# KhaoulaAguech/pl-fem-vectoriel

Hardware: AMD Instinct MI355X
Metric: eigenmodes/sec (assembly+solve), 7-core P2 mesh, 10 modes; |Δn_eff| vs ref (higher is better)
Workload: dtype f64

## Files before the change

pl_fem_vectoriel_amd/csrc/api_device.hip:

```cpp
#include <algorithm>
#include <atomic>
#include <memory>
#include <cmath>
#include <cstdio>
#include <cstdlib>
#include <cstring>
#include <chrono>
#include <mutex>
#include <numeric>
#include <thread>
#include <vector>

#include "device.h"
#include "host_eig.h"
#include "p2_element.h"

using plfem::Symbolic;

namespace {
template <class T>
T& process_wide() {
  static T* t = new T();
  return *t;
}
// ... 523 lines not shown
  if (!c) return PLFEM_EINVAL;
  if (!c->assembled) { c->err = "plfem_factor before plfem_assemble_hfield"; return PLFEM_ESTATE; }
  HIP_TRY(c, hipSetDevice(c->device));
  TRY(wait_for_upload(c));
  HIP_TRY(c, phase_begin(c, plfem::PH_FACTOR));
  HIP_TRY(c, hipMemsetAsync(c->d_fvec, 0, sizeof(double) * 2 * c->fnodes_total * plfem::BLOCK_P, c->stream));
  plfem::launch_factor(c, sigma);
  if (c->test_post_factor) c->test_post_factor(c);
  HIP_TRY(c, phase_end(c, plfem::PH_FACTOR));
  TRY(check_launch(c, "factor"));
  c->sigma = sigma;
  c->factored = true;
  return PLFEM_OK;
} catch (...) { return host_failure(c); }

extern "C" int plfem_solve(plfem_ctx* c, const double* rhs_dev, double* x_dev, int32_t refine_steps) try {
  if (!c || !rhs_dev || !x_dev || refine_steps < 0) return PLFEM_EINVAL;
  if (!c->factored) { c->err = "plfem_solve before plfem_factor"; return PLFEM_ESTATE; }
  HIP_TRY(c, hipSetDevice(c->device));
  plfem::solve_refined(c, 1, rhs_dev, x_dev, c->n2, false, refine_steps, c->d_t1, c->d_t2, c->d_t2);
  return check_launch(c, "solve");
} catch (...) { return host_failure(c); }

namespace {
struct ThickRestart {
  plfem_ctx* c;
  int P, k, ld;
  double tol;
  double* hH;
  std::vector<double> T, Tm, theta, Svec;
  std::vector<int> order;
  int nconv = 0, restarts = 0;
  double max_rel_res = 0.0;

  ThickRestart(plfem_ctx* c_, int P_, int k_, int m, double tol_)
      : c(c_), P(P_), k(k_), ld(m + P_), tol(tol_), hH(c_->h_pinned + plfem::PIN_PROJ), T((size_t)ld * ld, 0.0) {}

  void fill_tm(int mm) {
    Tm.assign((size_t)mm * mm, 0.0);
    for (int j = 0; j < mm; ++j)
      for (int i = 0; i <= j; ++i) {
        const double v = T[(size_t)j * ld + i];
        Tm[(size_t)j * mm + i] = v;
        Tm[(size_t)i * mm + j] = v;
      }
  }
  template <class Last>
  void count_converged(int mm, Last last) {
    order.resize(mm);
    std::iota(order.begin(), order.end(), 0);
    std::sort(order.begin(), order.end(), [&](int a, int b) { return std::fabs(theta[a]) > std::fabs(theta[b]); });
    nconv = 0;
    max_rel_res = 0.0;
    for (int q = 0; q < std::min(k, mm); ++q) {
      const int id = order[q];
      double res;
      if (P == 1) {
        res = std::fabs(T[(size_t)(mm - 1) * ld + mm] * last(id, 0));
      } else {
        double r2 = 0.0;
        for (int a = 0; a < P; ++a) {
          double v = 0.0;
          for (int b = a; b < P; ++b) v += T[(size_t)(mm - P + b) * ld + (mm + a)] * last(id, b);
          r2 += v * v;
        }
        res = std::sqrt(r2);
// ... 29 lines not shown
    std::swap(c->d_BV, c->d_BV2);
    std::fill(T.begin(), T.end(), 0.0);
    for (int q = 0; q < pk; ++q) T[(size_t)q * ld + q] = theta[order[q]];
    HIP_TRY(c, hipMemsetAsync(c->d_Hcols, 0, sizeof(double) * ld * ld, st));
    ++restarts;
    return PLFEM_OK;
  }

  int finish(int mm, double sigma, double* evals_host, double* evecs_dev, double* stats_host, int nop, int nblock) {
    hipStream_t st = c->stream;
    std::vector<int> want(order.begin(), order.begin() + k);
    std::vector<double> lam(mm);
    for (int i = 0; i < mm; ++i) lam[i] = sigma + 1.0 / theta[i];
    std::sort(want.begin(), want.end(), [&](int a, int b) { return lam[a] < lam[b]; });
    bool purify = nconv >= k;
    for (int a = 0; a < P; ++a) purify = purify && T[(size_t)(mm - P + a) * ld + (mm + a)] > 0.0;
    const int rows = purify ? mm + P : mm;
    for (int q = 0; q < k; ++q) {
      const int id = want[q];
      evals_host[q] = lam[id];
      double* s = hH + (size_t)q * rows;
      std::memcpy(s, &Svec[(size_t)id * mm], sizeof(double) * mm);
      for (int a = 0; a < rows - mm; ++a) {
        double v = 0.0;
        for (int b = a; b < P; ++b) v += T[(size_t)(mm - P + b) * ld + (mm + a)] * Svec[(size_t)id * mm + (mm - P + b)];
        s[mm + a] = v / theta[id];
      }
    }
    HIP_TRY(c, hipMemcpyAsync(c->d_S, hH, sizeof(double) * rows * k, hipMemcpyHostToDevice, st));
    if (!evecs_dev) evecs_dev = c->d_V2;
    c->modes_dev = evecs_dev;
    c->modes_k = k;
    plfem::launch_rotate(c, c->d_V, rows, c->d_S, rows, k, evecs_dev);
    HIP_TRY(c, phase_end(c, plfem::PH_LANCZOS));
    TRY(check_launch(c, "ritz rotation"));
    if (!c->defer_sync) HIP_TRY(c, hipStreamSynchronize(st));
    if (stats_host) {
      const double s[5] = {(double)nconv, (double)nop, (double)restarts, max_rel_res, (double)nblock};
      std::copy(s, s + 5, stats_host);
    }
    if (nconv < k) { c->err = "Lanczos: no convergence within maxiter restarts"; return PLFEM_ENOCONV; }
    return PLFEM_OK;
  }
};
}

static int lanczos_block(plfem_ctx* c, int k, int ncv, double tol, int maxiter, double sigma, double* evals_host,
                         double* evecs_dev, double* stats_host) {
  constexpr int P = plfem::BLOCK_P;
  const int64_t n = c->n2;
  hipStream_t st = c->stream;
  HIP_TRY(c, phase_begin(c, plfem::PH_LANCZOS));
  int m = ((ncv + P - 1) / P) * P;
  if (m > c->max_ncv) m = (c->max_ncv / P) * P;
  ThickRestart R(c, P, k, m, tol);
  const int ld = R.ld;
  int nop = 0, nblock = 0;
  {
    plfem::launch_start_field(c, P, c->d_V2);
    plfem::launch_spmv(c, 1, P, c->d_V2, c->d_bw, n);
    plfem::launch_solve(c, P, c->d_bw, c->d_w, n);
    nop += P; ++nblock;
    plfem::launch_spmv(c, 1, P, c->d_w, c->d_bw, n);
    plfem::launch_panel_dot(c, P, c->d_w, P, c->d_bw, n, c->d_G, P);
    plfem::launch_chol_block(c, c->d_G, P, c->d_hblk, P, c->d_Rinv);
    plfem::launch_block_scale(c, c->d_w, c->d_bw, n, c->d_Rinv, c->d_V, c->d_BV, n, nullptr, 0, nullptr, nullptr, c->d_fvec);
// ... 59 lines not shown
      R.ritz(mm_);
      return;
    }
    R.fill_tm(mm_);
    plfem::sym_band_eigenvalues(mm_, P, R.Tm.data(), mm_, R.theta);
    std::vector<int> ids(mm_);
    std::iota(ids.begin(), ids.end(), 0);
    std::sort(ids.begin(), ids.end(), [&](int a, int b) { return std::fabs(R.theta[a]) > std::fabs(R.theta[b]); });
    ids.resize(std::min(k, mm_));
    R.Svec.resize((size_t)mm_ * mm_);
    plfem::sym_band_eigenvectors(mm_, P, R.Tm.data(), mm_, R.theta, ids, R.Svec.data(), mm_);
    R.count_from_svec(mm_);
  };
  double res_prev = 0.0, res_last = 0.0;
  while (true) {
    int pend_c0 = -1, pend_slot = 0, slot = 0;
    bool converged = false, inflight = false, force_launch = false, have_full = false;
    mm = c0;
    while (true) {
      const bool predicted = !force_launch && pend_c0 >= 0 && res_prev > 0.0 && res_last > 0.0 &&
                             res_last * (res_last / res_prev) <= tol;
      force_launch = false;
      int new_c0 = -1, new_slot = 0;
      if (c0 + P <= m && !predicted) {
        TRY(launch_step(c0, slot));
        nop += P; ++nblock;
        new_c0 = c0; new_slot = slot;
        c0 += P; slot ^= 1;
      }
      if (pend_c0 >= 0) {
        TRY(absorb_step(pend_c0, pend_slot));
        mm = pend_c0 + P;
        if (mm >= k + P && (new_c0 >= 0 || predicted)) {
          if (predicted) { full_check(mm, false); have_full = true; } else { quick_check(mm); have_full = false; }
          res_prev = res_last;
          res_last = R.max_rel_res;
          if (getenv("PLFEM_LANCZOS_TRACE"))
            fprintf(stderr, "[lanczos] cols %d nconv %d max_rel_res %.3e%s\n", mm, R.nconv, R.max_rel_res, predicted ? " (held)" : "");
          if (R.nconv >= k) { converged = true; inflight = new_c0 >= 0; break; }
        }
        if (predicted) {
          pend_c0 = -1;
          force_launch = true;
          if (c0 + P <= m) continue;
          break;
        }
      }
      pend_c0 = new_c0; pend_slot = new_slot;
      if (pend_c0 < 0) break;
    }
    if (converged) {
      if (!have_full) full_check(mm, false);
      if (R.nconv < k) {
        converged = false;
        if (inflight) { TRY(absorb_step(c0 - P, slot ^ 1)); }
        res_prev = res_last = 0.0;
        if (c0 + P <= m) continue;
        mm = c0;
        full_check(mm, true);
      }
    } else {
      mm = c0;
      full_check(mm, true);
    }
    res_prev = res_last = 0.0;
    if (R.nconv >= k || R.restarts >= maxiter) break;
    int pk = 0;
    TRY(R.restart(mm, pk));
    c0 = pk;
    cycle_start = pk;
    il_ready = -1;
// ... 74 lines not shown
  if (!c || !evals_host || !evecs_dev) return PLFEM_EINVAL;
  return lanczos_run(c, k, ncv, tol, maxiter, sigma, evals_host, evecs_dev, stats_host);
} catch (...) { return host_failure(c); }

extern "C" int plfem_postprocess(plfem_ctx* c, int32_t k, double* evecs_dev, const double* cores_host, int32_t ncore,
                                 double* out_host, double* frac_core_host, double* modes_int_dev) try {
  if (!c || !evecs_dev || !out_host || k < 1 || k > c->max_ncv) return PLFEM_EINVAL;
  if (!c->assembled) { c->err = "plfem_postprocess before plfem_assemble_hfield"; return PLFEM_ESTATE; }
  HIP_TRY(c, hipSetDevice(c->device));
  TRY(upload_cores(c, cores_host, ncore));
  HIP_TRY(c, phase_begin(c, plfem::PH_POST));
  plfem::launch_post(c, k, evecs_dev, ncore, out_host, frac_core_host, modes_int_dev);
  HIP_TRY(c, phase_end(c, plfem::PH_POST));
  TRY(check_launch(c, "postprocess"));
  HIP_TRY(c, hipStreamSynchronize(c->stream));
  return PLFEM_OK;
} catch (...) { return host_failure(c); }

extern "C" int plfem_solve_modes(plfem_ctx* c, const double* cores_host, int32_t ncore, double eps_core, double eps_clad,
                                 double k0, double alpha_p, double sigma, int32_t k, int32_t ncv, double tol,
                                 int32_t maxiter, double residual_tol, double tol_refined, double* evals_host,
                                 double* post_host, double* frac_core_host, double* resid_host, double* modes_int_host,
                                 double* stats_host) try {
  if (!c || !evals_host || !post_host || !resid_host) return PLFEM_EINVAL;
  if (k < 1 || k > c->max_ncv) { c->err = "plfem_solve_modes: need 1 <= k <= max_ncv"; return PLFEM_EINVAL; }
  const double th0 = now_ms();
  HIP_TRY(c, hipSetDevice(c->device));
  if (!c->copy_stream) HIP_TRY(c, copy_stream_acquire(c->device, &c->copy_stream));
  if (!c->ev_copy) HIP_TRY(c, ctx_event_acquire(c->device, EV_NO_TIMING, &c->ev_copy));
  struct Defer {
    plfem_ctx* c;
    int saved_refine;
    bool copy_pending = false;
    hipEvent_t tr_ev[3] = {nullptr, nullptr, nullptr};
    ~Defer() {
      if (copy_pending) (void)hipStreamSynchronize(c->copy_stream);
      for (hipEvent_t e : tr_ev) if (e) (void)hipEventDestroy(e);
      c->defer_sync = false;
      c->refine_steps = saved_refine;
    }
  } defer{c, c->refine_steps};
  c->defer_sync = true;
  static const bool call_trace = getenv("PLFEM_CALL_TRACE") != nullptr;
  auto& tr_ev = defer.tr_ev;
  double th_asm = 0, th_fac = 0, th_lan = 0, th_enq = 0, th_sync = 0;
  if (call_trace) {
    for (auto& e : tr_ev) (void)hipEventCreate(&e);
    (void)hipEventRecord(tr_ev[0], c->stream);
  }
  if (c->dpn == 2) TRY(plfem_assemble_hfield(c, cores_host, ncore, eps_core, eps_clad, k0, alpha_p));
  else TRY(plfem_assemble_scalar(c, cores_host, ncore, eps_core, eps_clad, k0));
  th_asm = now_ms();
  TRY(plfem_factor(c, sigma));
  th_fac = now_ms();
  double st[8] = {0, 0, 0, 0, 0, 0, 0, 0};
  double first_res = 0.0, res = 0.0;
  int perturbed = 0, refined = 0;
  double n_opinv = 0, n_block = 0, restarts = 0;
  auto put_stats = [&](int lo, int hi) {
    if (!stats_host) return;
    double v[PLFEM_SOLVE_STATS] = {st[0], n_opinv, restarts, st[3], n_block, first_res, res, (double)refined, (double)perturbed};
    if (hi > PLFEM_SOLVE_T_ASSEMBLE_US) {
      for (int ph = 0; ph < plfem::PH_COUNT; ++ph) v[PLFEM_SOLVE_T_ASSEMBLE_US + ph] = phase_us(c, (plfem::Phase)ph);
      v[PLFEM_SOLVE_T_CALL_US] = (now_ms() - th0) * 1e3;
    }
    for (int q = lo; q < hi; ++q) stats_host[q] = v[q];
  };
  for (int pass = 0; pass < 2; ++pass) {
    c->refine_steps = pass == 0 ? defer.saved_refine : std::max(1, defer.saved_refine + 1);
    const double tol_p = pass == 0 ? tol : std::min(tol, tol_refined);
    const int rc = lanczos_run(c, k, ncv, tol_p, maxiter, sigma, evals_host, nullptr, st);
    n_opinv += st[1]; n_block += st[4]; restarts += st[2];
    if (rc != PLFEM_OK) {
      (void)hipStreamSynchronize(c->stream);
      put_stats(0, PLFEM_SOLVE_RESIDUAL_FIRST);
      return rc;
    }
    th_lan = now_ms();
    double* modes = c->modes_dev;
    double* modes_int = c->d_BV2 != modes ? c->d_BV2 : c->d_BV;
    HIP_TRY(c, phase_begin(c, plfem::PH_POST));
    hipError_t copy_err = hipSuccess;
    const size_t row_bytes = sizeof(double) * (size_t)c->dpn * c->nsolve;
    const std::function<void(int, int)> send_group = [&](int g0, int kg) {
      if (copy_err != hipSuccess) return;
      defer.copy_pending = true;
      copy_err = hipEventRecord(c->ev_copy, c->stream);
      if (copy_err == hipSuccess) copy_err = hipStreamWaitEvent(c->copy_stream, c->ev_copy, 0);
      if (copy_err == hipSuccess)
        copy_err = hipMemcpyAsync(reinterpret_cast<char*>(modes_int_host) + g0 * row_bytes, reinterpret_cast<char*>(modes_int) + g0 * row_bytes,
                                  kg * row_bytes, hipMemcpyDeviceToHost, c->copy_stream);
    };
    plfem::post_enqueue(c, k, modes, ncore, modes_int_host ? modes_int : nullptr, modes_int_host ? &send_group : nullptr);
    HIP_TRY(c, phase_end(c, plfem::PH_POST));
    HIP_TRY(c, copy_err);
    HIP_TRY(c, phase_begin(c, plfem::PH_RESIDUAL));
    plfem::resid_enqueue(c, k, evals_host, modes);
    HIP_TRY(c, phase_end(c, plfem::PH_RESIDUAL));
    TRY(check_launch(c, "post-processing + residual check"));
    if (call_trace) {
      (void)hipEventRecord(tr_ev[1], c->stream);
      (void)hipEventRecord(tr_ev[2], c->copy_stream);
    }
    th_enq = now_ms();
    HIP_TRY(c, hipStreamSynchronize(c->stream));
    th_sync = now_ms();
    plfem::post_finish(c, k, post_host, frac_core_host);
    plfem::resid_finish(c, k, resid_host);
    perturbed = reinterpret_cast<const int32_t*>(c->h_pinned + plfem::PIN_COUNTERS)[0];
    res = 0.0;
    for (int i = 0; i < k; ++i) res = (resid_host[i] > res || !(resid_host[i] == resid_host[i])) ? resid_host[i] : res;
    if (pass == 0) first_res = res;
    if (res <= residual_tol && perturbed == 0) break;
    if (modes_int_host) HIP_TRY(c, hipStreamSynchronize(c->copy_stream));
    defer.copy_pending = false;
    if (pass == 1) {
      if (res <= residual_tol) break;
      char msg[512];
      std::snprintf(msg, sizeof(msg), "eigen-residual %.2e after the refined re-run (first pass %.2e, bound %.0e); %s", res, first_res,
                    residual_tol, perturbed > 0 ? "vanishing pivots were perturbed: the shift-invert factorisation is inaccurate on this mesh"
                                                : "no pivot was perturbed: the eigenpairs did not converge tightly enough");
      c->err = msg;
      put_stats(PLFEM_SOLVE_RESIDUAL_FIRST, PLFEM_SOLVE_T_ASSEMBLE_US);
      return PLFEM_ERESIDUAL;
    }
    refined = 1;
  }
  if (modes_int_host) HIP_TRY(c, hipStreamSynchronize(c->copy_stream));
  defer.copy_pending = false;
  if (call_trace) {
    const double th_end = now_ms();
    float backlog = 0, total = 0, copy_tail = 0;
    (void)hipEventElapsedTime(&backlog, tr_ev[0], c->ev[plfem::PH_ASSEMBLE][0]);
    (void)hipEventElapsedTime(&total, tr_ev[0], tr_ev[1]);
    (void)hipEventElapsedTime(&copy_tail, tr_ev[1], tr_ev[2]);
    fprintf(stderr, "[call] host: assemble enqueued +%.3f, factor +%.3f, lanczos returned +%.3f, post + check enqueued +%.3f, stream done +%.3f, "
                    "copy done +%.3f ms | device: entry -> assembly %.3f (backlog of plfem_create + launch), entry -> end of check %.3f, "
                    "check -> copy end %.3f ms\n",
            th_asm - th0, th_fac - th0, th_lan - th0, th_enq - th0, th_sync - th0, th_end - th0, backlog, total, copy_tail);
  }
  put_stats(0, PLFEM_SOLVE_STATS);
  return PLFEM_OK;
} catch (...) { return host_failure(c); }

extern "C" int plfem_modes_dev(plfem_ctx* c, const double** evecs_dev, int32_t* k) try {
  if (!c || !evecs_dev) return PLFEM_EINVAL;
  if (!c->modes_dev) { c->err = "plfem_modes_dev: no eigen-solve has run on this context"; return PLFEM_ESTATE; }
  *evecs_dev = c->modes_dev;
  if (k) *k = c->modes_k;
  return PLFEM_OK;
} catch (...) { return host_failure(c); }

extern "C" int plfem_timings(plfem_ctx* c, double* out_host) try {
  if (!c || !out_host) return PLFEM_EINVAL;
  HIP_TRY(c, hipStreamSynchronize(c->stream));
  int32_t cnt[4] = {0, 0, 0, 0};
  HIP_TRY(c, hipMemcpy(cnt, c->d_counters, sizeof(cnt), hipMemcpyDeviceToHost));
  for (int ph = plfem::PH_ASSEMBLE; ph <= plfem::PH_UPLOAD; ++ph) out_host[ph] = phase_us(c, (plfem::Phase)ph);
  out_host[5] = cnt[0];
  out_host[6] = phase_us(c, plfem::PH_RESIDUAL);
  out_host[7] = 0.0;
  return PLFEM_OK;
} catch (...) { return host_failure(c); }

extern "C" int plfem_profile_begin(plfem_ctx* c, int32_t max_ranges) try {
  if (!c || max_ranges < 1) return PLFEM_EINVAL;
  HIP_TRY(c, hipSetDevice(c->device));
  c->prof_max = max_ranges;
  if (c->prof_ev.empty()) process_wide<EventPool>().take_all(c->device, EV_PROFILE, c->prof_ev);
  c->prof_n = 0;
  c->prof_toggle = 0;
  c->prof_slot.clear();
// ... 48 lines not shown
```

pl_fem_vectoriel_amd/csrc/host_eig.cpp:

```cpp
#include "host_eig.h"

#include <cmath>
#include <algorithm>
#include <cstddef>
#include <cstdint>
#include <numeric>
#include <utility>

namespace plfem {

namespace {

bool ql_implicit(int n, double* w, double* e, double* Z, int np) {
  auto zrow = [&](int i) -> double* { return Z + (size_t)i * np; };
  for (int i = 1; i < n; ++i) e[i - 1] = e[i];
  e[n - 1] = 0.0;
  bool ok = true;
  for (int l = 0; l < n; ++l) {
    int iter = 0, m;
    do {
      for (m = l; m < n - 1; ++m) {
        double dd = std::fabs(w[m]) + std::fabs(w[m + 1]);
        if (std::fabs(e[m]) <= 2.3e-16 * dd) break;
      }
// ... 2 lines not shown
        double gq = (w[l + 1] - w[l]) / (2.0 * e[l]);
        double r = std::hypot(gq, 1.0);
        gq = w[m] - w[l] + e[l] / (gq + (gq >= 0.0 ? std::fabs(r) : -std::fabs(r)));
        double s = 1.0, c = 1.0, pp = 0.0;
        int i;
        for (i = m - 1; i >= l; --i) {
          double f = s * e[i], b = c * e[i];
          e[i + 1] = (r = std::sqrt(f * f + gq * gq));
          if (r == 0.0) {
            w[i + 1] -= pp;
            e[m] = 0.0;
            break;
          }
          s = f / r;
          c = gq / r;
          gq = w[i + 1] - pp;
          r = (w[i] - gq) * s + 2.0 * c * b;
          w[i + 1] = gq + (pp = s * r);
          gq = c * r - b;
          double* z0 = zrow(i);
          double* z1 = zrow(i + 1);
          for (int k = 0; k < np; ++k) {
            const double f1 = z1[k], f0 = z0[k];
            z1[k] = s * f0 + c * f1;
            z0[k] = c * f0 - s * f1;
          }
        }
        if (r == 0.0 && i >= l) continue;
        w[l] -= pp;
        e[l] = gq;
        e[m] = 0.0;
      }
    } while (m != l);
  }
  return ok;
}

bool sym_eig_impl(int n, int last, std::vector<double>& A, std::vector<double>& V, std::vector<double>& w) {
  std::vector<double> e(n, 0.0), p(n, 0.0), g(n, 0.0), Yt;
  w.assign(n, 0.0);
  if (last < 0) V.swap(A);
  double* Z = last < 0 ? V.data() : A.data();
  auto row = [&](int i) -> double* { return Z + (size_t)i * n; };
  for (int i = n - 1; i > 0; --i) {
    const int l = i - 1;
    double* zi = row(i);
    double h = 0.0, scale = 0.0;
    if (l > 0) {
      for (int k = 0; k <= l; ++k) scale += std::fabs(zi[k]);
      if (scale == 0.0) {
        e[i] = zi[l];
      } else {
        for (int k = 0; k <= l; ++k) { zi[k] /= scale; h += zi[k] * zi[k]; }
        double f = zi[l];
        double gg = (f >= 0.0) ? -std::sqrt(h) : std::sqrt(h);
        e[i] = scale * gg;
        h -= f * gg;
        zi[l] = f - gg;
        for (int j = 0; j <= l; ++j) p[j] = 0.0;
        for (int j = 0; j <= l; ++j) {
          const double* zj = row(j);
          const double uj = zi[j];
          double s = 0.0;
          for (int k = 0; k < j; ++k) { s += zj[k] * zi[k]; p[k] += zj[k] * uj; }
          p[j] += s + zj[j] * uj;
        }
// ... 98 lines not shown
    }
    rp[p] = c * c * app + 2.0 * c * s_ * apq + s_ * s_ * aqq;
    rq[q] = s_ * s_ * app - 2.0 * c * s_ * apq + c * c * aqq;
    rp[q] = rq[p] = c * s_ * (aqq - app) + (c * c - s_ * s_) * apq;
    for (int k = lo; k <= hi; ++k) {
      at(k, p) = rp[k];
      at(k, q) = rq[k];
    }
  };
  auto annihilate = [&](int r, int col) {
    const double x = at(r - 1, col), y = at(r, col);
    if (y == 0.0) return false;
    const double h = std::sqrt(x * x + y * y);
    rotate(r - 1, x / h, y / h, col, std::min(n - 1, r + b));
    at(r, col) = 0.0;
    at(col, r) = 0.0;
    return true;
  };
  for (int j = 0; j + 2 < n; ++j)
    for (int d = std::min(b, n - 1 - j); d >= 2; --d) {
      int r = j + d;
      if (!annihilate(r, j)) continue;
      while (r + b < n) {
        const int col = r - 1;
        r += b;
        if (!annihilate(r, col)) break;
      }
    }
  w.resize(n);
  for (int i = 0; i < n; ++i) {
    w[i] = at(i, i);
    e[i] = i > 0 ? at(i, i - 1) : 0.0;
  }
  const bool ok = ql_implicit(n, w.data(), e.data(), nullptr, 0);
  std::sort(w.begin(), w.end());
  return ok;
}

bool sym_band_eigenvectors(int n, int b, const double* A, int lda, const std::vector<double>& w, const std::vector<int>& ids,
                           double* S, int lds) {
  const double eps = 2.220446049250313e-16;
  double anorm = 0.0;
  for (int i = 0; i < n; ++i) {
    double rs = 0.0;
    for (int j = std::max(0, i - b); j <= std::min(n - 1, i + b); ++j) rs += std::fabs(A[(size_t)std::min(i, j) * lda + std::max(i, j)]);
    anorm = std::max(anorm, rs);
  }
  if (anorm == 0.0) anorm = 1.0;
  const double sep = 10.0 * eps * anorm, ortol = 1e-3 * anorm, tiny = eps * anorm;
  std::vector<int> seq(ids);
  std::sort(seq.begin(), seq.end(), [&](int x, int y) { return w[x] < w[y] || (w[x] == w[y] && x < y); });
  std::vector<double> M((size_t)n * n, 0.0), x(n), y(n);
  std::vector<int> piv(n);
  auto at = [&](int i, int j) -> double& { return M[(size_t)i * n + j]; };
  bool ok = true;
  double lam_prev = 0.0, w_prev = 0.0;
  size_t cluster0 = 0;
  uint64_t rng = 0x2545F4914F6CDD1Dull;
  for (size_t t = 0; t < seq.size(); ++t) {
    const int id = seq[t];
    double lam = w[id];
    if (t > 0) {
      if (w[id] - w_prev > ortol) cluster0 = t;
      if (lam - lam_prev < sep) lam = lam_prev + sep;
    }
    lam_prev = lam;
    w_prev = w[id];
    for (int i = 0; i < n; ++i) {
      for (int j = std::max(0, i - b); j <= std::min(n - 1, i + 2 * b); ++j) at(i, j) = 0.0;
      for (int j = std::max(0, i - b); j <= std::min(n - 1, i + b); ++j) at(i, j) = A[(size_t)std::min(i, j) * lda + std::max(i, j)];
      at(i, i) -= lam;
    }
    for (int c = 0; c < n; ++c) {
      const int rmax = std::min(n - 1, c + b), cmax = std::min(n - 1, c + 2 * b);
      int pr = c;
      for (int r = c + 1; r <= rmax; ++r)
        if (std::fabs(at(r, c)) > std::fabs(at(pr, c))) pr = r;
      piv[c] = pr;
      if (pr != c)
        for (int k = c; k <= cmax; ++k) std::swap(at(c, k), at(pr, k));
      if (std::fabs(at(c, c)) < tiny) at(c, c) = at(c, c) < 0.0 ? -tiny : tiny;
      for (int r = c + 1; r <= rmax; ++r) {
        const double l = at(r, c) / at(c, c);
        at(r, c) = l;
        if (l != 0.0)
          for (int k = c + 1; k <= cmax; ++k) at(r, k) -= l * at(c, k);
      }
    }
    for (int i = 0; i < n; ++i) {
      rng = rng * 6364136223846793005ull + 1442695040888963407ull;
      x[i] = ((double)(rng >> 11) / 9007199254740992.0) * 2.0 - 1.0;
    }
    const double want_growth = 1.0 / (100.0 * std::sqrt((double)n) * eps * anorm);
    int extra = -1;
    for (int it = 0; it < 8 && extra != 0; ++it) {
      double nx = 0.0;
      for (int i = 0; i < n; ++i) nx += x[i] * x[i];
      nx = std::sqrt(nx);
      for (int i = 0; i < n; ++i) y[i] = x[i] / nx;
      for (int c = 0; c < n; ++c) {
        if (piv[c] != c) std::swap(y[c], y[piv[c]]);
        const double yc = y[c];
        for (int r = c + 1; r <= std::min(n - 1, c + b); ++r) y[r] -= at(r, c) * yc;
      }
      for (int c = n - 1; c >= 0; --c) {
        double v = y[c];
        for (int k = c + 1; k <= std::min(n - 1, c + 2 * b); ++k) v -= at(c, k) * y[k];
        y[c] = v / at(c, c);
      }
      double growth = 0.0;
      for (int i = 0; i < n; ++i) growth += y[i] * y[i];
      growth = std::sqrt(growth);
      for (size_t u = cluster0; u < t; ++u) {
        const double* v = S + (size_t)seq[u] * lds;
        double dot = 0.0;
        for (int i = 0; i < n; ++i) dot += v[i] * y[i];
        for (int i = 0; i < n; ++i) y[i] -= dot * v[i];
      }
      x.swap(y);
      if (extra > 0) --extra;
      else if (extra < 0 && growth >= want_growth) extra = 2;
    }
    if (extra < 0) ok = false;
    double nx = 0.0;
    for (int i = 0; i < n; ++i) nx += x[i] * x[i];
    nx = 1.0 / std::sqrt(nx);
    double* out = S + (size_t)id * lds;
    for (int i = 0; i < n; ++i) out[i] = x[i] * nx;
  }
  return ok;
}

}
```

pl_fem_vectoriel_amd/csrc/kernels_lanczos.hip:

```cpp
#include <algorithm>
#include <cmath>
#include <functional>

#include "device.h"
#include "p2_element.h"

namespace plfem {
namespace {

typedef double v4d __attribute__((ext_vector_type(4)));
constexpr int CHUNK = PANEL_CHUNK;

__global__ __launch_bounds__(256) void k_scale_store(int64_t n, const double* __restrict__ w,
                                                     const double* __restrict__ bw, const double* __restrict__ beta2,
                                                     double* __restrict__ v, double* __restrict__ bv,
                                                     double* __restrict__ beta_out) {
  const double b2 = *beta2;
  const double beta = sqrt(fmax(b2, 0.0));
  const double inv = beta > 0.0 ? 1.0 / beta : 0.0;
  const int64_t i = (int64_t)blockIdx.x * 256 + threadIdx.x;
  if (i == 0 && beta_out) *beta_out = beta;
  if (i >= n) return;
  v[i] = w[i] * inv;
  bv[i] = bw[i] * inv;
// ... 393 lines not shown
      for (int j = 0; j < MB; ++j) {
        double ux = vx[j][c], uy = vx[j][yoff + c];
        px[j] += a * ux + 2.0 * b * uy;
        py[j] += d * uy;
      }
    }
    const bool msk = mask[row] != 0;
#pragma unroll
    for (int j = 0; j < MB; ++j) {
      double x = vx[j][row], y = DPN == 2 ? vx[j][yoff + row] : 0.0;
      acc[j][4] += x * px[j] + y * py[j];
      if (sub == 0) {
        acc[j][0] += x * x;
        acc[j][1] += y * y;
        if (msk) { acc[j][2] += x * x; acc[j][3] += y * y; }
      }
    }
  }
#pragma unroll
  for (int j = 0; j < MB; ++j)
#pragma unroll
    for (int t = 0; t < 5; ++t) {
      double v = acc[j][t];
      for (int off = 32; off >= 1; off >>= 1) v += __shfl_xor(v, off);
      if ((threadIdx.x & 63) == 0) red[threadIdx.x >> 6][j][t] = v;
    }
  __syncthreads();
  if ((int)threadIdx.x < 5 * nm) {
    const int j = threadIdx.x / 5, t = threadIdx.x % 5;
    partial[((int64_t)(mode0 + j) * nblocks + blockIdx.x) * 5 + t] = red[0][j][t] + red[1][j][t] + red[2][j][t] + red[3][j][t];
  }
}

__global__ __launch_bounds__(64) void k_post_finish(int k, int nblocks, const double* __restrict__ partial,
                                                    double* __restrict__ out) {
  const int t = blockIdx.x;
  const int mode = t / 5, q = t % 5;
  double acc = 0.0;
  for (int b = threadIdx.x; b < nblocks; b += 64) acc += partial[((int64_t)mode * nblocks + b) * 5 + q];
  for (int off = 32; off >= 1; off >>= 1) acc += __shfl_xor(acc, off);
  if (threadIdx.x == 0) out[t] = acc;
}

__global__ __launch_bounds__(256) void k_post_scale(int N, int dpn, const double* __restrict__ sums, double* __restrict__ evecs) {
  const int mode = blockIdx.y;
  const double n2 = dpn == 2 ? sums[mode * 5 + 0] + sums[mode * 5 + 1] : sums[mode * 5 + 4];
  const double nrm = sqrt(n2) + 1e-30;
  const double inv = 1.0 / nrm;
  double* v = evecs + (int64_t)mode * dpn * N;
  const int64_t i = (int64_t)blockIdx.x * 256 + threadIdx.x;
  if (i < dpn * (int64_t)N) v[i] *= inv;
}

__global__ __launch_bounds__(256) void k_gather_interior(int N, int nsolve, int dpn, const int32_t* __restrict__ interior,
                                                         const double* __restrict__ evecs,
                                                         double* __restrict__ modes_int) {
  const int mode = blockIdx.y;
  const int64_t i = (int64_t)blockIdx.x * 256 + threadIdx.x;
  if (i >= dpn * (int64_t)nsolve) return;
  int comp = i >= nsolve ? 1 : 0;
  int q = (int)(i - (int64_t)comp * nsolve);
  modes_int[(int64_t)mode * dpn * nsolve + i] = evecs[(int64_t)mode * dpn * N + (int64_t)comp * N + interior[q]];
}

template <int DPN>
__global__ __launch_bounds__(256) void k_resid_sums(int N, int k, int nblocks, const int32_t* __restrict__ rowptr,
                                                    const int32_t* __restrict__ colind, const uint8_t* __restrict__ bmask,
                                                    const double* __restrict__ vxx, const double* __restrict__ vxy,
                                                    const double* __restrict__ vyx, const double* __restrict__ vyy,
                                                    const double* __restrict__ vm, const double* __restrict__ lam,
                                                    const double* __restrict__ evecs, double* __restrict__ partial) {
  constexpr int MB = POST_MB;
  const int mode0 = blockIdx.y * MB;
  const int nm = min(MB, k - mode0);
  const double* vx[MB];
  double l[MB];
#pragma unroll
  for (int j = 0; j < MB; ++j) {
    const int mode = min(mode0 + j, k - 1);
    vx[j] = evecs + (int64_t)mode * DPN * N;
    l[j] = lam[mode];
  }
  const int64_t yoff = DPN == 2 ? N : 0;
  __shared__ double red[4][MB][2];
  double r2[MB], a2[MB];
#pragma unroll
  for (int j = 0; j < MB; ++j) { r2[j] = 0.0; a2[j] = 0.0; }
  const int sub = threadIdx.x & 7;
  for (int rr = threadIdx.x >> 3; rr < POST_ROWS; rr += 32) {
    const int row = blockIdx.x * POST_ROWS + rr;
    if (row >= N) break;
    if (bmask[row]) continue;
    double ax[MB], ay[MB], bx[MB], by[MB];
#pragma unroll
    for (int j = 0; j < MB; ++j) { ax[j] = 0; ay[j] = 0; bx[j] = 0; by[j] = 0; }
// ... 158 lines not shown
    cm *= cm;
    k >>= 1;
  }
  const uint64_t s = am * 0x9E3779B97F4A7C15ull + ap;
  const int q = (int)(e / (dpn * (int64_t)nsolve));
  const int r = (int)(e - (int64_t)q * dpn * nsolve);
  const int comp = r >= nsolve, i = r - comp * nsolve;
  out[(int64_t)q * ld + (int64_t)comp * N + interior[i]] = ((double)(s >> 11) / 9007199254740992.0) * 2.0 - 1.0;
}

void launch_start_field(plfem_ctx* c, int nvec, double* out) {
  (void)hipMemsetAsync(out, 0, sizeof(double) * c->n2 * nvec, c->stream);
  const int64_t total = (int64_t)nvec * c->dpn * c->nsolve;
  hipLaunchKernelGGL(k_start_field, dim3((unsigned)((total + 255) / 256)), dim3(256), 0, c->stream, c->nsolve, c->N, c->dpn,
                     c->n2, nvec, c->d_interior, out);
}

void launch_rotate(plfem_ctx* c, const double* V, int m, const double* Smat, int ldS, int p, double* out) {
  const int mpad = (m + 3) & ~3;
  const int chunk = std::max(16, ((64 * 1024) / (8 * mpad)) & ~15);
  unsigned grid = (unsigned)((c->n2 + 63) / 64);
  for (int p0 = 0; p0 < p; p0 += chunk) {
    const int pc = std::min(chunk, p - p0);
    const size_t lds = sizeof(double) * mpad * ((pc + 15) & ~15);
    hipLaunchKernelGGL(k_rotate, dim3(grid), dim3(256), lds, c->stream, c->n2, m, pc, V, Smat + (size_t)p0 * ldS, ldS,
                       out + (size_t)p0 * c->n2);
  }
}

constexpr int POST_GROUP = 8;
void post_enqueue(plfem_ctx* c, int k, double* evecs, int ncore, double* modes_int, const std::function<void(int, int)>* group_done) {
  hipStream_t st = c->stream;
  const int N = c->N;
  (void)hipMemsetAsync(c->d_counters + 1, 0, sizeof(int32_t), st);
  hipLaunchKernelGGL(k_core_mask, dim3((N + 255) / 256), dim3(256), 0, st, N, c->d_doflocs, c->d_cores, ncore,
                     c->d_bmask, c->d_coremask, c->d_counters);
  const int nblocks = post_blocks(N);
  const int group = group_done ? POST_GROUP : k;
  for (int g0 = 0; g0 < k; g0 += group) {
    const int kg = std::min(group, k - g0);
    double* ev = evecs + (int64_t)g0 * c->n2;
    double* partial = c->d_post + (int64_t)g0 * nblocks * POST_SUMS;
    double* sums = c->d_post + (int64_t)k * nblocks * POST_SUMS + (int64_t)g0 * POST_SUMS;
    const double* dxx = c->d_vals[c->dpn == 1 ? PLFEM_BLK_MINV : PLFEM_BLK_DXX];
    with_constant<1, 2>(c->dpn, [&](auto dpn) {
      hipLaunchKernelGGL(k_post_sums<decltype(dpn)::value>, dim3(nblocks, (kg + POST_MB - 1) / POST_MB), dim3(256), 0, st, N, kg, nblocks,
                         c->d_rowptr, c->d_colind, dxx, c->d_vals[PLFEM_BLK_DXY], c->d_vals[PLFEM_BLK_DYY], c->d_coremask, ev, partial);
    });
    hipLaunchKernelGGL(k_post_finish, dim3(kg * POST_SUMS), dim3(64), 0, st, kg, nblocks, partial, sums);
    hipLaunchKernelGGL(k_post_scale, dim3((unsigned)((c->n2 + 255) / 256), kg), dim3(256), 0, st, N, c->dpn, sums, ev);
    if (modes_int)
      hipLaunchKernelGGL(k_gather_interior, dim3((unsigned)((c->dpn * (int64_t)c->nsolve + 255) / 256), kg), dim3(256), 0, st,
                         N, c->nsolve, c->dpn, c->d_interior, ev, modes_int + (int64_t)g0 * c->dpn * c->nsolve);
    if (group_done) (*group_done)(g0, kg);
  }
  double* hs = c->h_pinned + PIN_POST;
  (void)hipMemcpyAsync(hs, c->d_post + (int64_t)k * nblocks * POST_SUMS, sizeof(double) * k * POST_SUMS, hipMemcpyDeviceToHost, st);
  int32_t* hc = reinterpret_cast<int32_t*>(c->h_pinned + PIN_COUNTERS);
  (void)hipMemcpyAsync(hc, c->d_counters, sizeof(int32_t) * 4, hipMemcpyDeviceToHost, st);
}

void post_finish(plfem_ctx* c, int k, double* out_host, double* frac_core) {
  const double* hs = c->h_pinned + PIN_POST;
  const int32_t* hc = reinterpret_cast<const int32_t*>(c->h_pinned + PIN_COUNTERS);
  for (int mode = 0; mode < k; ++mode) {
    const double* s = hs + mode * POST_SUMS;
    double nrm2 = c->dpn == 2 ? s[0] + s[1] : s[4];
    double nrm = std::sqrt(nrm2) + 1e-30;
    double inv2 = 1.0 / (nrm * nrm);
    double* o = out_host + (size_t)mode * PLFEM_POST_COUNT;
    o[PLFEM_POST_NORM] = nrm;
    o[PLFEM_POST_DIV_ENERGY] = s[4] * inv2;
    o[PLFEM_POST_CORE_X] = s[2] * inv2;
    o[PLFEM_POST_CORE_Y] = s[3] * inv2;
    o[PLFEM_POST_ALL_X] = s[0] * inv2;
    o[PLFEM_POST_ALL_Y] = s[1] * inv2;
  }
  if (frac_core) *frac_core = (double)hc[1] / (double)c->nsolve;
}

void launch_post(plfem_ctx* c, int k, double* evecs, int ncore, double* out_host, double* frac_core,
                 double* modes_int) {
  post_enqueue(c, k, evecs, ncore, modes_int, nullptr);
// ... 6 lines not shown
```

Baseline: 520.0.

## Start interior mode copy early, root-free QL, banded inverse iteration storage

The post-processing now computes mode norms with a dedicated reduction and gathers normalized interior modes before the full post sums. This lets the device-to-host copy start earlier and overlap the remaining post kernels. On the host, tridiagonal eigenvalues now use a root-free QL variant, and inverse iteration stores only the band instead of a dense n×n matrix, with reciprocal pivots and unrolled norms. The change also adds trace timing output, and it duplicates a normalization that must stay consistent with k_post_scale.

```diff
diff --git a/pl_fem_vectoriel_amd/csrc/api_device.hip b/pl_fem_vectoriel_amd/csrc/api_device.hip
--- a/pl_fem_vectoriel_amd/csrc/api_device.hip
+++ b/pl_fem_vectoriel_amd/csrc/api_device.hip
@@ -579,6 +579,7 @@
   std::vector<int> order;
   int nconv = 0, restarts = 0;
   double max_rel_res = 0.0;
+  double t_held = 0.0;
 
   ThickRestart(plfem_ctx* c_, int P_, int k_, int m, double tol_)
       : c(c_), P(P_), k(k_), ld(m + P_), tol(tol_), hH(c_->h_pinned + plfem::PIN_PROJ), T((size_t)ld * ld, 0.0) {}
@@ -674,6 +675,8 @@
     c->modes_dev = evecs_dev;
     c->modes_k = k;
     plfem::launch_rotate(c, c->d_V, rows, c->d_S, rows, k, evecs_dev);
+    if (t_held > 0.0)
+      fprintf(stderr, "[lanczos] held step absorbed -> rotation enqueued: %.1f us on the host\n", (now_ms() - t_held) * 1e3);
     HIP_TRY(c, phase_end(c, plfem::PH_LANCZOS));
     TRY(check_launch(c, "ritz rotation"));
     if (!c->defer_sync) HIP_TRY(c, hipStreamSynchronize(st));
@@ -799,11 +802,16 @@
         TRY(absorb_step(pend_c0, pend_slot));
         mm = pend_c0 + P;
         if (mm >= k + P && (new_c0 >= 0 || predicted)) {
+          const bool trace = getenv("PLFEM_LANCZOS_TRACE") != nullptr;
+          const double t_check = trace ? now_ms() : 0.0;
           if (predicted) { full_check(mm, false); have_full = true; } else { quick_check(mm); have_full = false; }
           res_prev = res_last;
           res_last = R.max_rel_res;
-          if (getenv("PLFEM_LANCZOS_TRACE"))
-            fprintf(stderr, "[lanczos] cols %d nconv %d max_rel_res %.3e%s\n", mm, R.nconv, R.max_rel_res, predicted ? " (held)" : "");
+          if (trace) {
+            fprintf(stderr, "[lanczos] cols %d nconv %d max_rel_res %.3e%s (host test %.1f us)\n", mm, R.nconv, R.max_rel_res,
+                    predicted ? " (held)" : "", (now_ms() - t_check) * 1e3);
+            R.t_held = predicted ? t_check : 0.0;
+          }
           if (R.nconv >= k) { converged = true; inflight = new_c0 >= 0; break; }
         }
         if (predicted) {
@@ -944,7 +952,7 @@
     plfem_ctx* c;
     int saved_refine;
     bool copy_pending = false;
-    hipEvent_t tr_ev[3] = {nullptr, nullptr, nullptr};
+    hipEvent_t tr_ev[4] = {nullptr, nullptr, nullptr, nullptr};
     ~Defer() {
       if (copy_pending) (void)hipStreamSynchronize(c->copy_stream);
       for (hipEvent_t e : tr_ev) if (e) (void)hipEventDestroy(e);
@@ -999,6 +1007,7 @@
       defer.copy_pending = true;
       copy_err = hipEventRecord(c->ev_copy, c->stream);
       if (copy_err == hipSuccess) copy_err = hipStreamWaitEvent(c->copy_stream, c->ev_copy, 0);
+      if (call_trace && g0 == 0) (void)hipEventRecord(tr_ev[3], c->copy_stream);
       if (copy_err == hipSuccess)
         copy_err = hipMemcpyAsync(reinterpret_cast<char*>(modes_int_host) + g0 * row_bytes, reinterpret_cast<char*>(modes_int) + g0 * row_bytes,
                                   kg * row_bytes, hipMemcpyDeviceToHost, c->copy_stream);
@@ -1042,14 +1051,15 @@
   defer.copy_pending = false;
   if (call_trace) {
     const double th_end = now_ms();
-    float backlog = 0, total = 0, copy_tail = 0;
+    float backlog = 0, total = 0, copy_tail = 0, copy_start = 0;
     (void)hipEventElapsedTime(&backlog, tr_ev[0], c->ev[plfem::PH_ASSEMBLE][0]);
     (void)hipEventElapsedTime(&total, tr_ev[0], tr_ev[1]);
     (void)hipEventElapsedTime(&copy_tail, tr_ev[1], tr_ev[2]);
+    if (modes_int_host) (void)hipEventElapsedTime(&copy_start, c->ev[plfem::PH_LANCZOS][1], tr_ev[3]);
     fprintf(stderr, "[call] host: assemble enqueued +%.3f, factor +%.3f, lanczos returned +%.3f, post + check enqueued +%.3f, stream done +%.3f, "
                     "copy done +%.3f ms | device: entry -> assembly %.3f (backlog of plfem_create + launch), entry -> end of check %.3f, "
-                    "check -> copy end %.3f ms\n",
-            th_asm - th0, th_fac - th0, th_lan - th0, th_enq - th0, th_sync - th0, th_end - th0, backlog, total, copy_tail);
+                    "check -> copy end %.3f, lanczos end -> first copy start %.3f ms\n",
+            th_asm - th0, th_fac - th0, th_lan - th0, th_enq - th0, th_sync - th0, th_end - th0, backlog, total, copy_tail, copy_start);
   }
   put_stats(0, PLFEM_SOLVE_STATS);
   return PLFEM_OK;
diff --git a/pl_fem_vectoriel_amd/csrc/host_eig.cpp b/pl_fem_vectoriel_amd/csrc/host_eig.cpp
--- a/pl_fem_vectoriel_amd/csrc/host_eig.cpp
+++ b/pl_fem_vectoriel_amd/csrc/host_eig.cpp
@@ -58,6 +58,61 @@
         e[m] = 0.0;
       }
     } while (m != l);
+  }
+  return ok;
+}
+
+bool ql_rootfree(int n, double* w, double* e) {
+  const double eps = 2.220446049250313e-16, eps2 = eps * eps;
+  for (int i = 1; i < n; ++i) e[i - 1] = e[i] * e[i];
+  e[n - 1] = 0.0;
+  bool ok = true;
+  int l = 0, iter = 0;
+  while (l < n) {
+    int m;
+    for (m = l; m < n - 1; ++m)
+      if (std::fabs(e[m]) <= eps2 * std::fabs(w[m] * w[m + 1])) break;
+    if (m < n - 1) e[m] = 0.0;
+    if (m == l) { ++l; iter = 0; continue; }
+    if (m == l + 1) {
+      const double a = w[l], b = std::sqrt(e[l]), c = w[l + 1];
+      const double sm = a + c, adf = std::fabs(a - c), ab = std::fabs(b + b);
+      const double acmx = std::fabs(a) > std::fabs(c) ? a : c, acmn = std::fabs(a) > std::fabs(c) ? c : a;
+      double rt;
+      if (adf > ab) rt = adf * std::sqrt(1.0 + (ab / adf) * (ab / adf));
+      else if (adf < ab) rt = ab * std::sqrt(1.0 + (adf / ab) * (adf / ab));
+      else rt = ab * std::sqrt(2.0);
+      double rt1, rt2;
+      if (sm < 0.0) { rt1 = 0.5 * (sm - rt); rt2 = (acmx / rt1) * acmn - (b / rt1) * b; }
+      else if (sm > 0.0) { rt1 = 0.5 * (sm + rt); rt2 = (acmx / rt1) * acmn - (b / rt1) * b; }
+      else { rt1 = 0.5 * rt; rt2 = -0.5 * rt; }
+      w[l] = rt1;
+      w[l + 1] = rt2;
+      e[l] = 0.0;
+      l += 2;
+      iter = 0;
+      continue;
+    }
+    if (iter++ == 120) { ok = false; ++l; iter = 0; continue; }
+    double p = w[l];
+    const double rte = std::sqrt(e[l]);
+    double sigma = (w[l + 1] - p) / (2.0 * rte);
+    const double r0 = std::hypot(sigma, 1.0);
+    sigma = p - rte / (sigma + (sigma >= 0.0 ? r0 : -r0));
+    double c = 1.0, s = 0.0, gamma = w[m] - sigma;
+    p = gamma * gamma;
+    for (int i = m - 1; i >= l; --i) {
+      const double bb = e[i], r = p + bb;
+      if (i != m - 1) e[i + 1] = s * r;
+      const double oldc = c, oldgam = gamma, alpha = w[i];
+      c = p / r;
+      s = bb / r;
+      gamma = c * (alpha - sigma) - s * oldgam;
+      w[i + 1] = oldgam + (alpha - gamma);
+      p = c != 0.0 ? (gamma * gamma) / c : oldc * bb;
+    }
+    e[l] = s * p;
+    w[l] = sigma + gamma;
   }
   return ok;
 }
@@ -222,9 +277,19 @@
     w[i] = at(i, i);
     e[i] = i > 0 ? at(i, i - 1) : 0.0;
   }
-  const bool ok = ql_implicit(n, w.data(), e.data(), nullptr, 0);
+  const bool ok = ql_rootfree(n, w.data(), e.data());
   std::sort(w.begin(), w.end());
   return ok;
+}
+
+namespace {
+double sum_sq(const double* v, int n) {
+  double s0 = 0.0, s1 = 0.0, s2 = 0.0, s3 = 0.0;
+  int i = 0;
+  for (; i + 4 <= n; i += 4) { s0 += v[i] * v[i]; s1 += v[i + 1] * v[i + 1]; s2 += v[i + 2] * v[i + 2]; s3 += v[i + 3] * v[i + 3]; }
+  for (; i < n; ++i) s0 += v[i] * v[i];
+  return (s0 + s1) + (s2 + s3);
+}
 }
 
 bool sym_band_eigenvectors(int n, int b, const double* A, int lda, const std::vector<double>& w, const std::vector<int>& ids,
@@ -240,9 +305,13 @@
   const double sep = 10.0 * eps * anorm, ortol = 1e-3 * anorm, tiny = eps * anorm;
   std::vector<int> seq(ids);
   std::sort(seq.begin(), seq.end(), [&](int x, int y) { return w[x] < w[y] || (w[x] == w[y] && x < y); });
-  std::vector<double> M((size_t)n * n, 0.0), x(n), y(n);
+  const int W = 3 * b + 1;
+  std::vector<double> B0((size_t)n * W, 0.0), M((size_t)n * W), x(n), y(n), rdiag(n);
   std::vector<int> piv(n);
-  auto at = [&](int i, int j) -> double& { return M[(size_t)i * n + j]; };
+  auto at = [&](int i, int j) -> double& { return M[(size_t)i * W + (j - i + b)]; };
+  for (int i = 0; i < n; ++i)
+    for (int j = std::max(0, i - b); j <= std::min(n - 1, i + b); ++j)
+      B0[(size_t)i * W + (j - i + b)] = A[(size_t)std::min(i, j) * lda + std::max(i, j)];
   bool ok = true;
   double lam_prev = 0.0, w_prev = 0.0;
   size_t cluster0 = 0;
@@ -256,11 +325,8 @@
     }
     lam_prev = lam;
     w_prev = w[id];
-    for (int i = 0; i < n; ++i) {
-      for (int j = std::max(0, i - b); j <= std::min(n - 1, i + 2 * b); ++j) at(i, j) = 0.0;
-      for (int j = std::max(0, i - b); j <= std::min(n - 1, i + b); ++j) at(i, j) = A[(size_t)std::min(i, j) * lda + std::max(i, j)];
-      at(i, i) -= lam;
-    }
+    M = B0;
+    for (int i = 0; i < n; ++i) at(i, i) -= lam;
     for (int c = 0; c < n; ++c) {
       const int rmax = std::min(n - 1, c + b), cmax = std::min(n - 1, c + 2 * b);
       int pr = c;
@@ -270,11 +336,14 @@
       if (pr != c)
         for (int k = c; k <= cmax; ++k) std::swap(at(c, k), at(pr, k));
       if (std::fabs(at(c, c)) < tiny) at(c, c) = at(c, c) < 0.0 ? -tiny : tiny;
+      const double* rc = &at(c, c);
+      rdiag[c] = 1.0 / rc[0];
       for (int r = c + 1; r <= rmax; ++r) {
-        const double l = at(r, c) / at(c, c);
-        at(r, c) = l;
+        double* rr = &at(r, c);
+        const double l = rr[0] * rdiag[c];
+        rr[0] = l;
         if (l != 0.0)
-          for (int k = c + 1; k <= cmax; ++k) at(r, k) -= l * at(c, k);
+          for (int k = 1; k <= cmax - c; ++k) rr[k] -= l * rc[k];
       }
     }
     for (int i = 0; i < n; ++i) {
@@ -284,23 +353,21 @@
     const double want_growth = 1.0 / (100.0 * std::sqrt((double)n) * eps * anorm);
     int extra = -1;
     for (int it = 0; it < 8 && extra != 0; ++it) {
-      double nx = 0.0;
-      for (int i = 0; i < n; ++i) nx += x[i] * x[i];
-      nx = std::sqrt(nx);
-      for (int i = 0; i < n; ++i) y[i] = x[i] / nx;
+      const double nx = 1.0 / std::sqrt(sum_sq(x.data(), n));
+      for (int i = 0; i < n; ++i) y[i] = x[i] * nx;
       for (int c = 0; c < n; ++c) {
         if (piv[c] != c) std::swap(y[c], y[piv[c]]);
         const double yc = y[c];
         for (int r = c + 1; r <= std::min(n - 1, c + b); ++r) y[r] -= at(r, c) * yc;
       }
       for (int c = n - 1; c >= 0; --c) {
+        const double* rc = &at(c, c);
+        const double* yc = &y[c];
         double v = y[c];
-        for (int k = c + 1; k <= std::min(n - 1, c + 2 * b); ++k) v -= at(c, k) * y[k];
-        y[c] = v / at(c, c);
-      }
-      double growth = 0.0;
-      for (int i = 0; i < n; ++i) growth += y[i] * y[i];
-      growth = std::sqrt(growth);
+        for (int k = std::min(n - 1, c + 2 * b) - c; k >= 1; --k) v -= rc[k] * yc[k];
+        y[c] = v * rdiag[c];
+      }
+      const double growth = std::sqrt(sum_sq(y.data(), n));
       for (size_t u = cluster0; u < t; ++u) {
         const double* v = S + (size_t)seq[u] * lds;
         double dot = 0.0;
@@ -312,9 +379,7 @@
       else if (extra < 0 && growth >= want_growth) extra = 2;
     }
     if (extra < 0) ok = false;
-    double nx = 0.0;
-    for (int i = 0; i < n; ++i) nx += x[i] * x[i];
-    nx = 1.0 / std::sqrt(nx);
+    const double nx = 1.0 / std::sqrt(sum_sq(x.data(), n));
     double* out = S + (size_t)id * lds;
     for (int i = 0; i < n; ++i) out[i] = x[i] * nx;
   }
diff --git a/pl_fem_vectoriel_amd/csrc/kernels_lanczos.hip b/pl_fem_vectoriel_amd/csrc/kernels_lanczos.hip
--- a/pl_fem_vectoriel_amd/csrc/kernels_lanczos.hip
+++ b/pl_fem_vectoriel_amd/csrc/kernels_lanczos.hip
@@ -449,10 +449,48 @@
   }
 }
 
-__global__ __launch_bounds__(64) void k_post_finish(int k, int nblocks, const double* __restrict__ partial,
+__global__ __launch_bounds__(256) void k_post_norm_sums(int N, int k, int nblocks, const double* __restrict__ evecs,
+                                                        double* __restrict__ partial) {
+  constexpr int MB = POST_MB;
+  const int mode0 = blockIdx.y * MB;
+  const int nm = min(MB, k - mode0);
+  const double* vx[MB];
+#pragma unroll
+  for (int j = 0; j < MB; ++j) vx[j] = evecs + (int64_t)min(mode0 + j, k - 1) * 2 * N;
+  __shared__ double red[4][MB][2];
+  double acc[MB][2];
+#pragma unroll
+  for (int j = 0; j < MB; ++j) { acc[j][0] = 0.0; acc[j][1] = 0.0; }
+  if ((threadIdx.x & 7) == 0)
+    for (int rr = threadIdx.x >> 3; rr < POST_ROWS; rr += 32) {
+      const int row = blockIdx.x * POST_ROWS + rr;
+      if (row >= N) break;
+#pragma unroll
+      for (int j = 0; j < MB; ++j) {
+        const double x = vx[j][row], y = vx[j][(int64_t)N + row];
+        acc[j][0] = fma(x, x, acc[j][0]);
+        acc[j][1] = fma(y, y, acc[j][1]);
+      }
+    }
+#pragma unroll
+  for (int j = 0; j < MB; ++j)
+#pragma unroll
+    for (int t = 0; t < 2; ++t) {
+      double v = acc[j][t];
+      for (int off = 32; off >= 1; off >>= 1) v += __shfl_xor(v, off);
+      if ((threadIdx.x & 63) == 0) red[threadIdx.x >> 6][j][t] = v;
+    }
+  __syncthreads();
+  if ((int)threadIdx.x < 2 * nm) {
+    const int j = threadIdx.x >> 1, t = threadIdx.x & 1;
+    partial[((int64_t)(mode0 + j) * nblocks + blockIdx.x) * 5 + t] = red[0][j][t] + red[1][j][t] + red[2][j][t] + red[3][j][t];
+  }
+}
+
+__global__ __launch_bounds__(64) void k_post_finish(int k, int nblocks, int nq, const double* __restrict__ partial,
                                                     double* __restrict__ out) {
-  const int t = blockIdx.x;
-  const int mode = t / 5, q = t % 5;
+  const int mode = blockIdx.x / nq, q = blockIdx.x % nq;
+  const int t = mode * 5 + q;
   double acc = 0.0;
   for (int b = threadIdx.x; b < nblocks; b += 64) acc += partial[((int64_t)mode * nblocks + b) * 5 + q];
   for (int off = 32; off >= 1; off >>= 1) acc += __shfl_xor(acc, off);
@@ -478,6 +516,20 @@
   int comp = i >= nsolve ? 1 : 0;
   int q = (int)(i - (int64_t)comp * nsolve);
   modes_int[(int64_t)mode * dpn * nsolve + i] = evecs[(int64_t)mode * dpn * N + (int64_t)comp * N + interior[q]];
+}
+
+__global__ __launch_bounds__(256) void k_gather_interior_scaled(int N, int nsolve, const int32_t* __restrict__ interior,
+                                                                const double* __restrict__ sums, const double* __restrict__ evecs,
+                                                                double* __restrict__ modes_int) {
+  const int mode = blockIdx.y;
+  const double n2 = sums[mode * 5 + 0] + sums[mode * 5 + 1];
+  const double nrm = sqrt(n2) + 1e-30;
+  const double inv = 1.0 / nrm;
+  const int64_t i = (int64_t)blockIdx.x * 256 + threadIdx.x;
+  if (i >= 2 * (int64_t)nsolve) return;
+  int comp = i >= nsolve ? 1 : 0;
+  int q = (int)(i - (int64_t)comp * nsolve);
+  modes_int[(int64_t)mode * 2 * nsolve + i] = evecs[(int64_t)mode * 2 * N + (int64_t)comp * N + interior[q]] * inv;
 }
 
 template <int DPN>
@@ -702,11 +754,24 @@
 void post_enqueue(plfem_ctx* c, int k, double* evecs, int ncore, double* modes_int, const std::function<void(int, int)>* group_done) {
   hipStream_t st = c->stream;
   const int N = c->N;
+  const int nblocks = post_blocks(N);
+  const int group = group_done ? POST_GROUP : k;
+  const bool early = c->dpn == 2 && modes_int;
+  if (early) {
+    double* sums = c->d_post + (int64_t)k * nblocks * POST_SUMS;
+    hipLaunchKernelGGL(k_post_norm_sums, dim3(nblocks, (k + POST_MB - 1) / POST_MB), dim3(256), 0, st, N, k, nblocks, evecs, c->d_post);
+    hipLaunchKernelGGL(k_post_finish, dim3(k * 2), dim3(64), 0, st, k, nblocks, 2, c->d_post, sums);
+    for (int g0 = 0; g0 < k; g0 += group) {
+      const int kg = std::min(group, k - g0);
+      hipLaunchKernelGGL(k_gather_interior_scaled, dim3((unsigned)((2 * (int64_t)c->nsolve + 255) / 256), kg), dim3(256), 0, st,
+                         N, c->nsolve, c->d_interior, sums + (int64_t)g0 * POST_SUMS, evecs + (int64_t)g0 * c->n2,
+                         modes_int + (int64_t)g0 * 2 * c->nsolve);
+      if (group_done) (*group_done)(g0, kg);
+    }
+  }
   (void)hipMemsetAsync(c->d_counters + 1, 0, sizeof(int32_t), st);
   hipLaunchKernelGGL(k_core_mask, dim3((N + 255) / 256), dim3(256), 0, st, N, c->d_doflocs, c->d_cores, ncore,
                      c->d_bmask, c->d_coremask, c->d_counters);
-  const int nblocks = post_blocks(N);
-  const int group = group_done ? POST_GROUP : k;
   for (int g0 = 0; g0 < k; g0 += group) {
     const int kg = std::min(group, k - g0);
     double* ev = evecs + (int64_t)g0 * c->n2;
@@ -717,8 +782,9 @@
       hipLaunchKernelGGL(k_post_sums<decltype(dpn)::value>, dim3(nblocks, (kg + POST_MB - 1) / POST_MB), dim3(256), 0, st, N, kg, nblocks,
                          c->d_rowptr, c->d_colind, dxx, c->d_vals[PLFEM_BLK_DXY], c->d_vals[PLFEM_BLK_DYY], c->d_coremask, ev, partial);
     });
-    hipLaunchKernelGGL(k_post_finish, dim3(kg * POST_SUMS), dim3(64), 0, st, kg, nblocks, partial, sums);
+    hipLaunchKernelGGL(k_post_finish, dim3(kg * POST_SUMS), dim3(64), 0, st, kg, nblocks, POST_SUMS, partial, sums);
     hipLaunchKernelGGL(k_post_scale, dim3((unsigned)((c->n2 + 255) / 256), kg), dim3(256), 0, st, N, c->dpn, sums, ev);
+    if (early) continue;
     if (modes_int)
       hipLaunchKernelGGL(k_gather_interior, dim3((unsigned)((c->dpn * (int64_t)c->nsolve + 255) / 256), kg), dim3(256), 0, st,
                          N, c->nsolve, c->dpn, c->d_interior, ev, modes_int + (int64_t)g0 * c->dpn * c->nsolve);
```

New measurement: 510.9. 0.983x the previous value.
